# seiya-kumada/3d_gaussian_splatting

Measured on AMD Instinct MI355X. Metric: forward+backward iters/s at 1080p, 1M Gaussians; PSNR vs CPU ref, higher is better.
Workload: dtype f32; 1 GPU; 1m_1080p: 1000000 Gaussians, 1920x1080, SH degree 3, fwd+bwd; gaussians=1000000, width=1920, height=1080, sh_degree=3, parallelism=single GPU

## Files before the change

### 3d_gaussian_splatting_amd/csrc/gsr_api.cpp

```cpp
#include <hip/hip_runtime.h>

#include <algorithm>
#include <climits>
#include <cstdlib>
#include <cstdarg>
#include <cstdio>
#include <cstring>
#include <mutex>
#include <string>
#include <vector>

#include "gsr_kernels.h"

using namespace gsr;

namespace {

thread_local std::string g_err;

struct PinnedWord {
    static constexpr int kWords = 256;
    volatile uint32_t* p = nullptr;
    PinnedWord() {
        void* q = nullptr;
// ... 265 lines not shown
        v.kA = at<uint32_t>(b->binning, bl.kA);
        v.vA = at<uint32_t>(b->binning, bl.vA);
        v.kB = at<uint32_t>(b->binning, bl.kB);
        v.vB = at<uint32_t>(b->binning, bl.vB);
        v.hist = at<uint32_t>(b->binning, bl.hist);
        v.mk = at<uint8_t>(b->binning, bl.mk);
        v.rb_histB = at<uint32_t>(b->binning, bl.rb_hist);
        const int tiles = div_up(cam->width, kTile) * div_up(cam->height, kTile);
        const bool odd = !v.rb && (tile_passes(tiles) & 1) != 0;
        v.sorted_tile = odd ? v.kB : v.kA;
        v.sorted_gid = odd ? v.vB : v.vA;
        v.free_k = odd ? v.kA : v.kB;
        v.free_v = odd ? v.vA : v.vB;
    }
    return v;
}

__global__ void fill_background(float* out_color, float* final_T, float* accum,
                                int npix, float bg0, float bg1, float bg2) {
    const int i = blockIdx.x * 256 + threadIdx.x;
    if (i >= npix) return;
    accum[i] = 0.0f;
    accum[npix + i] = 0.0f;
    accum[2 * (size_t)npix + i] = 0.0f;
    out_color[i] = bg0;
    out_color[npix + i] = bg1;
    out_color[2 * (size_t)npix + i] = bg2;
    final_T[i] = 1.0f;
}

struct FwdJob {
    const gsr_camera* cam;
    const gsr_raster_settings* rs;
    float* out_color;
    gsr_buffers* bufs;
    long long n = 0;
    int ty0 = 0, ty1 = 0, gx = 0, gy = 0;
    int vgy = 0, vh = 0;
    bool rows_counted = false;
    const gsr_aux_out* aux = nullptr;
    bool antialias() const { return (rs->flags & GSR_FLAG_ANTIALIAS) != 0; }
    uint32_t mode_bits() const {
        return (aux ? kBufAux | ((rs->flags & GSR_FLAG_INVDEPTH) ? kBufInvDepth : 0u) : 0u) |
               (antialias() ? kBufAntialias : 0u);
    }
};

template <class Pre>
int fwd_phase1(FwdJob& j, gsr_alloc_fn alloc_geom, gsr_alloc_fn alloc_image, void* ctx, hipStream_t stream, bool debug,
               bool band_pixels_only, Pre&& pre) {
    const gsr_camera* cam = j.cam;
    const gsr_raster_settings* rs = j.rs;
    gsr_buffers* bufs = j.bufs;
    const int W = cam->width, H = cam->height;
    j.gx = div_up(W, kTile);
    j.gy = div_up(H, kTile);
    band(cam, rs, &j.ty0, &j.ty1);
    std::memset(bufs, 0, sizeof *bufs);
    bufs->layout = GSR_LAYOUT_TAG | (use_presort(j.n, j.gx, j.gy) ? kBufPresort : 0u) | j.mode_bits();
    bufs->num_rendered = -1;
    bufs->n_local = (int32_t)j.n;
    bufs->geom = alloc_geom(ctx, GeomLayout(j.n).total);
    bufs->image = alloc_image(ctx, ImgLayout(W, H, j.aux != nullptr).total);
    if (!bufs->geom || !bufs->image) return fail(-2, "allocation failed (geometry/image)");
    const ImgLayout il(W, H);
    const Views v = views(cam, j.n, bufs);
    if ((j.ty0 > 0 || j.ty1 < j.gy) && !band_pixels_only) {
        const int npix = W * H;
        hipLaunchKernelGGL(fill_background, dim3(div_up(npix, 256)), dim3(256), 0, stream, j.out_color, v.final_T,
                           v.accum, npix, rs->bg[0], rs->bg[1], rs->bg[2]);
        GSR_STAGE(GSR_STAGE_MISC, hipGetLastError(), "fill_background");
    }
    GSR_STAGE(GSR_STAGE_MISC, hipMemsetAsync(v.ranges, 0, il.ovf - il.ranges, stream), "clear ranges");
    if (int e = pre(v)) return e;
    if (v.presort) {
        GSR_STAGE(GSR_STAGE_DEPTH_SORT, launch_depth_presort(v.depth_key, v.tiles, v.rect, (int)j.n, v.dk0, v.dv0,
                                                             v.dk1, v.dv1, v.dhist, v.rtiles, v.rrect, v.lookback,
                                                             v.K_dev, stream),
                  "depth presort");
        return 0;
    }
    const bool rb_possible = use_rb_binning(j.n, j.gx, j.gy);
    if (rb_possible && j.rows_counted)
        GSR_STAGE(GSR_STAGE_SCAN, launch_scan_blocks(v.lookback + 16, (int)j.n, v.K_dev, stream), "scan (block sums)");
    else
        GSR_STAGE(GSR_STAGE_SCAN, launch_scan(v.tiles, (int)j.n, v.offsets, v.partials, v.K_dev, stream, !rb_possible),
                  "scan");
    return 0;
}

int fwd_phase2(FwdJob& j, long long cap, gsr_alloc_fn alloc_binning, void* ctx, hipStream_t stream, bool debug) {
    const gsr_camera* cam = j.cam;
    gsr_buffers* bufs = j.bufs;
    if (cap > INT32_MAX) return fail(-3, "num_rendered overflow (%lld)", cap);
    bufs->capacity = (int32_t)cap;
    bufs->binning = alloc_binning(ctx, BinLayout(cap, (long long)ImgLayout::tile_count(cam->width, cam->height),
                                                 j.aux != nullptr).total);
    if (!bufs->binning) return fail(-2, "allocation failed (binning, %lld instances)", cap);
    const int tiles = j.gx * j.gy, ntiles = (j.ty1 - j.ty0) * j.gx;
    const bool scanned = use_rb_binning(j.n, j.gx, j.gy);
    bufs->layout = expected_layout(j.n, j.gx, j.gy, cap) | j.mode_bits();
    const Views v = views(cam, j.n, bufs);
    auto depth_sort = [&](bool unordered, const uint2* src) {
        return launch_tile_depth_sort(v.ranges, j.ty0 * j.gx, ntiles, cap, v.depth_key, v.sorted_gid, v.ovf,
                                      v.counters + kOvfCountSlot, v.ovf2, v.counters + kOvf2CountSlot, v.done,
                                      v.free_k, v.free_v, stream, unordered, src);
    };
    if (v.presort)
        GSR_STAGE(GSR_STAGE_DUPLICATE, launch_duplicate_ranked(v.rtiles, v.rrect, v.rect, (int)j.n, j.gx, j.ty0,
                                                               v.lookback, v.offsets, v.kA, v.vA, cap, stream),
                  "duplicate (rank order)");
    else if (!v.rb) {
        if (scanned && j.rows_counted)
            GSR_STAGE(GSR_STAGE_SCAN, launch_block_offsets(v.tiles, (int)j.n, v.lookback + 16, v.offsets, stream),
                      "offsets");
        GSR_STAGE(GSR_STAGE_DUPLICATE, launch_duplicate(v.tiles, v.rect, (int)j.n, j.gx, j.ty0, v.offsets, v.lookback,
                                                        v.kA, v.vA, cap, v.K_dev, stream, scanned),
                  "duplicate");
    }
    if (cap > 0 && v.rb) {
        const bool rb_keys = v.ck_bytes >= 4 * (size_t)cap;
        uint2* const ppair = rb_keys ? reinterpret_cast<uint2*>(v.kA) : nullptr;
        uint2* const tpair = rb_keys ? reinterpret_cast<uint2*>(v.kB) : nullptr;
        uint32_t* const pxr = rb_keys ? reinterpret_cast<uint32_t*>(v.ck) : v.vB;
        GSR_STAGE(GSR_STAGE_TILE_SORT, launch_rb_binning(v.tiles, v.rect, v.offsets, (int)j.n, j.gx, j.ty0, j.ty1,
                                                         v.rb_histA, v.rb_histB, v.rb_status, v.kB, pxr, v.vA,
                                                         v.ranges, cap, stream, j.rows_counted,
                                                         j.rows_counted ? v.lookback + 16 : nullptr, v.K_dev,
                                                         v.depth_key, ppair, tpair),
                  "row-bucketed binning");
        GSR_STAGE(GSR_STAGE_DEPTH_SORT, depth_sort(true, tpair), "per-tile depth order");
    } else if (cap > 0) {
        int which = -1;
        GSR_STAGE(GSR_STAGE_TILE_SORT, radix_sort(v.kA, v.vA, v.kB, v.vB, v.kA, v.vA, cap, v.K_dev, tile_bits(tiles),
                                                  v.hist, &which, stream),
                  "tile sort");
        if ((which == 0) != (v.sorted_tile == v.kB)) return fail(-12, "tile sort ended in an unexpected buffer");
        GSR_STAGE(GSR_STAGE_FINALIZE, launch_finalize(v.sorted_tile, cap, v.K_dev, v.ranges, stream), "finalize");
        if (!v.presort) GSR_STAGE(GSR_STAGE_DEPTH_SORT, depth_sort(false, nullptr), "per-tile depth order");
    }
    F6Aux f6{};
    if (j.aux)
        f6 = {v.depth_key, j.aux->depth, j.aux->alpha, v.accum_z, v.ckz, (j.rs->flags & GSR_FLAG_INVDEPTH) ? 1 : 0};
    GSR_STAGE(GSR_STAGE_BLEND_FWD, launch_blend_forward(*cam, j.rs->bg, j.ty0, j.ty1, v.ranges, v.sorted_gid, v.rec,
                                                        j.out_color, v.final_T, v.accum, v.term, v.ck, cap, stream,
                                                        j.vgy, j.vh, v.mk, j.aux ? &f6 : nullptr),
              j.aux ? "blend forward (aux)" : "blend forward");
    return 0;
}

int fwd_sized_phase2(FwdJob& j, gsr_alloc_fn alloc_binning, void* ctx, hipStream_t stream, bool debug) {
    long long cap = j.rs->max_rendered;
    if (cap == 0) {
        uint64_t ksum = 0;
        if (j.n > 0) {
            uint32_t cw[2 * kCountSlots];
            const Views v = views(j.cam, j.n, j.bufs);
            GSR_STAGE(GSR_STAGE_MISC, end_read(v.counters, cw, 2 * kCountSlots, stream), "read counts");
            for (int i = 0; i < kCountSlots; ++i) ksum += cw[kCountSlots + i];
        }
        if (ksum > (uint64_t)INT32_MAX) return fail(-3, "num_rendered overflow (%llu)", (unsigned long long)ksum);
        cap = (long long)ksum;
        j.bufs->num_rendered = (int32_t)ksum;
    }
    return fwd_phase2(j, cap, alloc_binning, ctx, stream, debug);
}

// ... 680 lines not shown
```

### 3d_gaussian_splatting_amd/csrc/gsr_binning.hip

```cpp
#include "gsr_kernels.h"
#include "gsr_sort_dev.h"

namespace gsr {
namespace {

constexpr int kB = kSortBlock;
constexpr int kI = kSortItems;
constexpr int kWaves = kB / 64;

__device__ inline uint32_t block_exclusive_scan(uint32_t v, uint32_t* wsum, uint32_t* total) {
    const int tid = threadIdx.x, w = tid >> 6, lane = tid & 63;
    uint32_t x = v;
#pragma unroll
    for (int o = 1; o < 64; o <<= 1) {
        const uint32_t y = __shfl_up(x, o, 64);
        if (lane >= o) x += y;
    }
    if (lane == 63) wsum[w] = x;
    __syncthreads();
    uint32_t pre = 0, tot = 0;
    const int nw = blockDim.x >> 6;
    for (int k = 0; k < nw; ++k) {
        pre += (k < w) ? wsum[k] : 0u;
        tot += wsum[k];
// ... 1 lines not shown
    __syncthreads();
    *total = tot;
    return pre + x - v;
}

__global__ __launch_bounds__(kB) void scan_reduce(const uint32_t* __restrict__ in, int n,
                                                  uint32_t* __restrict__ partials) {
    __shared__ uint32_t wsum[kWaves];
    const int base = blockIdx.x * kSortTile;
    uint32_t s = 0;
#pragma unroll
    for (int r = 0; r < kI; ++r) {
        const int i = base + r * kB + threadIdx.x;
        if (i < n) s += in[i];
    }
    uint32_t tot;
    block_exclusive_scan(s, wsum, &tot);
    if (threadIdx.x == 0) partials[blockIdx.x] = tot;
}

constexpr int kScanQ = 8, kScanQ1 = 32;
__device__ __forceinline__ uint32_t wide_block_scan(uint32_t* __restrict__ a, int n, uint32_t* wsum) {
    uint32_t carry = 0;
    for (int base = 0; base < n; base += 1024 * kScanQ) {
        const int i0 = base + (int)threadIdx.x * kScanQ;
        uint32_t v[kScanQ], sv = 0;
#pragma unroll
        for (int q = 0; q < kScanQ; ++q) {
            v[q] = i0 + q < n ? a[i0 + q] : 0u;
            sv += v[q];
        }
        uint32_t tot;
        uint32_t run = carry + block_exclusive_scan(sv, wsum, &tot);
#pragma unroll
        for (int q = 0; q < kScanQ; ++q) {
            if (i0 + q < n) a[i0 + q] = run;
            run += v[q];
        }
        carry += tot;
    }
    return carry;
}

__device__ __forceinline__ uint32_t wide_block_scan_lds(uint32_t* __restrict__ a, int n, uint32_t* wsum,
                                                        uint32_t* buf) {
    for (int i = (int)threadIdx.x; i < n; i += 1024) buf[i] = a[i];
    __syncthreads();
    const int Q = (n + 1023) / 1024;
    const int i0 = (int)threadIdx.x * Q;
    uint32_t v[kScanQ1], sv = 0;
#pragma unroll
    for (int q = 0; q < kScanQ1; ++q) {
        v[q] = q < Q && i0 + q < n ? buf[i0 + q] : 0u;
        sv += v[q];
    }
    uint32_t tot;
    uint32_t run = block_exclusive_scan(sv, wsum, &tot);
#pragma unroll
    for (int q = 0; q < kScanQ1; ++q) {
        if (q < Q && i0 + q < n) buf[i0 + q] = run;
        run += v[q];
    }
    __syncthreads();
    for (int i = (int)threadIdx.x; i < n; i += 1024) a[i] = buf[i];
    return tot;
}
__host__ __device__ constexpr bool scan_lds_fits(long long n) { return n <= 1024LL * kScanQ1; }

__global__ __launch_bounds__(1024) void scan_partials(uint32_t* __restrict__ partials, int nb,
                                                      uint32_t* __restrict__ total_out) {
    extern __shared__ uint32_t sbuf[];
    __shared__ uint32_t wsum[16];
    const uint32_t carry = scan_lds_fits(nb) ? wide_block_scan_lds(partials, nb, wsum, sbuf)
                                             : wide_block_scan(partials, nb, wsum);
    if (threadIdx.x == 0 && total_out) *total_out = carry;
}

__global__ __launch_bounds__(1024) void rb_colscan(uint32_t* __restrict__ hist, int nb, uint32_t* __restrict__ totals) {
    extern __shared__ uint32_t sbuf[];
    __shared__ uint32_t wsum[16];
    uint32_t* const a = hist + (size_t)blockIdx.x * nb;
    const uint32_t carry = scan_lds_fits(nb) ? wide_block_scan_lds(a, nb, wsum, sbuf) : wide_block_scan(a, nb, wsum);
    if (threadIdx.x == 0) totals[blockIdx.x] = carry;
}
static size_t scan_lds_bytes(long long n) { return scan_lds_fits(n) ? sizeof(uint32_t) * (size_t)n : 0; }

__global__ __launch_bounds__(kB) void scan_downsweep(const uint32_t* __restrict__ in, int n,
                                                     const uint32_t* __restrict__ partials,
                                                     uint32_t* __restrict__ out) {
    __shared__ uint32_t buf[kSortTile + kSortTile / 32];
    __shared__ uint32_t wsum[kWaves];
    const int base = blockIdx.x * kSortTile;
    const int tid = threadIdx.x;
    auto pad = [](int i) { return i + (i >> 5); };
#pragma unroll
    for (int r = 0; r < kI; ++r) {
        const int i = r * kB + tid;
        const int g = base + i;
        buf[pad(i)] = g < n ? in[g] : 0u;
    }
    __syncthreads();
    uint32_t v[kI];
    uint32_t s = 0;
#pragma unroll
    for (int k = 0; k < kI; ++k) {
        v[k] = buf[pad(tid * kI + k)];
        s += v[k];
        v[k] = s;
    }
    uint32_t tot;
    const uint32_t ex = block_exclusive_scan(s, wsum, &tot) + partials[blockIdx.x];
#pragma unroll
    for (int k = 0; k < kI; ++k) buf[pad(tid * kI + k)] = v[k] + ex;
    __syncthreads();
#pragma unroll
    for (int r = 0; r < kI; ++r) {
        const int i = r * kB + tid;
        if (base + i < n) out[base + i] = buf[pad(i)];
    }
}

__device__ __forceinline__ uint32_t udiv_small(uint32_t a, uint32_t b) {
    return (uint32_t)(((float)a + 0.5f) * __builtin_amdgcn_rcpf((float)b));
}

__device__ __forceinline__ void emit_wave(const uint32_t* s_start, const uint32_t* s_g, const uint32_t* s_w,
                                          const uint32_t* s_x0, const uint32_t* s_y0, uint32_t first,
                                          uint32_t wtotal, int grid_x, long long cap, uint32_t* __restrict__ tkey,
                                          uint32_t* __restrict__ tgid) {
    const int lane = threadIdx.x & 63;
    for (uint32_t i = lane; i < wtotal; i += 64) {
        if ((long long)first + i >= cap) break;
        int o = 0;
#pragma unroll
        for (int step = 32; step > 0; step >>= 1)
            if (s_start[o + step] <= i) o += step;
        const uint32_t local = i - s_start[o];
        const uint32_t wd = s_w[o];
        const uint32_t dy = udiv_small(local, wd), dx = local - dy * wd;
        tkey[first + i] = (s_y0[o] + dy) * (uint32_t)grid_x + s_x0[o] + dx;
        tgid[first + i] = s_g[o];
    }
}

constexpr uint32_t kAgg = 1u << 30, kInc = 2u << 30, kCntMask = kAgg - 1u;

__global__ __launch_bounds__(256) void scan_duplicate_kernel(const uint32_t* __restrict__ tiles,
                                                             uint4* __restrict__ rect, int n,
                                                             int grid_x, int ty0,
                                                             uint32_t* __restrict__ offsets,
                                                             uint32_t* __restrict__ tkey,
                                                             uint32_t* __restrict__ tgid, long long cap,
                                                             uint32_t* __restrict__ status,
                                                             uint32_t* __restrict__ ticket,
                                                             uint32_t* __restrict__ total_out) {
    __shared__ uint32_t s_start[kWaves][64], s_g[kWaves][64], s_w[kWaves][64], s_x0[kWaves][64],
        s_y0[kWaves][64];
    __shared__ uint32_t wsum[kWaves];
    __shared__ uint32_t s_excl;
    __shared__ int s_b;
    const int tid = threadIdx.x, w = tid >> 6, lane = tid & 63;
    if (tid == 0) s_b = (int)atomicAdd(ticket, 1u);
    __syncthreads();
    const int b = s_b;
    const int g = b * 256 + tid;
    const bool valid = g < n;
// ... 77 lines not shown
                                                        const uint32_t* __restrict__ tiles,
                                                        uint4* __restrict__ rect, const uint4* __restrict__ rrect,
                                                        int P, int grid_x, int ty0,
                                                        uint32_t* __restrict__ tkey, uint32_t* __restrict__ tgid,
                                                        long long cap, const uint32_t* __restrict__ bexcl) {
    __shared__ uint32_t s_start[kWaves][64], s_g[kWaves][64], s_w[kWaves][64], s_x0[kWaves][64],
        s_y0[kWaves][64];
    __shared__ uint32_t wsum[kWaves];
    const int tid = threadIdx.x, w = tid >> 6, lane = tid & 63;
    const int i = blockIdx.x * 256 + tid;
    const bool valid = i < P;
    uint32_t nt = 0, end = 0, g = (uint32_t)i;
    if (RANKED) {
        if (valid) nt = tiles[i];
        uint32_t tot;
        end = bexcl[blockIdx.x] + block_exclusive_scan(nt, wsum, &tot) + nt;
        if (valid) offsets[i] = end;
    } else if (valid) {
        nt = tiles[i];
        end = offsets[i];
    }
    uint32_t minx = 0, maxx = 0, y0 = 0;
    if (nt) {
        uint4 rr;
        if (RANKED) {
            rr = rrect[i];
            g = rr.z;
            rect[g].z = end - nt;
        } else {
            rect[g].z = end - nt;
            rr = rect[g];
        }
        minx = rr.x & 0xFFFF;
        maxx = rr.y & 0xFFFF;
        const uint32_t miny = rr.x >> 16;
        y0 = miny > (uint32_t)ty0 ? miny : (uint32_t)ty0;
    }
    const uint32_t first = (uint32_t)__builtin_amdgcn_readfirstlane((int)(end - nt));
    const uint64_t vmask = __ballot(valid);
    if (vmask == 0) return;
    const int last_lane = 63 - __builtin_clzll(vmask);
    const uint32_t total = (uint32_t)__builtin_amdgcn_readlane((int)end, last_lane) - first;
    s_start[w][lane] = valid ? end - nt - first : 0xFFFFFFFFu;
    s_g[w][lane] = g;
    s_w[w][lane] = maxx - minx;
    s_x0[w][lane] = minx;
    s_y0[w][lane] = y0;
    wave_lds_sync();
    emit_wave(s_start[w], s_g[w], s_w[w], s_x0[w], s_y0[w], first, total, grid_x, cap, tkey, tgid);
}

__global__ __launch_bounds__(256) void rank_payload_kernel(const uint32_t* __restrict__ sgid,
                                                           const uint32_t* __restrict__ tiles,
                                                           const uint4* __restrict__ rect, int n,
                                                           uint32_t* __restrict__ rtiles,
                                                           uint4* __restrict__ rrect, uint32_t* __restrict__ bsum) {
    __shared__ uint32_t wsum[kWaves];
    const int r = blockIdx.x * 256 + threadIdx.x;
    uint32_t nt = 0;
    if (r < n) {
        const uint32_t g = sgid[r];
        nt = tiles[g];
        uint4 q = make_uint4(0u, 0u, g, 0u);
        if (nt) {
            const uint4 rr = rect[g];
            q.x = rr.x;
            q.y = rr.y;
        }
        rtiles[r] = nt;
        rrect[r] = q;
    }
    uint32_t s = nt;
#pragma unroll
    for (int o = 32; o > 0; o >>= 1) s += __shfl_xor(s, o, 64);
    if ((threadIdx.x & 63) == 0) wsum[threadIdx.x >> 6] = s;
    __syncthreads();
    if (threadIdx.x == 0) bsum[blockIdx.x] = wsum[0] + wsum[1] + wsum[2] + wsum[3];
}

constexpr int kRbChunk = kRbChunkPairs;
static_assert(kRbChunk % 256 == 0 && kRbMaxRows == 256 && kRbMaxCols == 256, "one row / column per thread");
constexpr int kRbStageA = 1024;
constexpr int kRbStage = 4096;

__global__ __launch_bounds__(256) void rb_rows_count(const uint32_t* __restrict__ tiles, const uint4* __restrict__ rect,
                                                     int n, int ty0, int ty1, uint32_t* __restrict__ histA, int nbA) {
    __shared__ uint32_t cnt[kRbMaxRows];
    const int tid = threadIdx.x, R = ty1 - ty0;
    cnt[tid] = 0u;
    __syncthreads();
    const int g = blockIdx.x * 256 + tid;
    if (g < n) {
        const uint32_t nt = tiles[g];
        if (nt) {
            const uint4 rr = rect[g];
            const int miny = (int)(rr.x >> 16), maxy = (int)(rr.y >> 16);
            const int by0 = miny > ty0 ? miny : ty0, by1 = maxy < ty1 ? maxy : ty1;
            for (int r = by0; r < by1; ++r) atomicAdd(&cnt[r - ty0], 1u);
        }
    }
    __syncthreads();
    if (tid < R) histA[(size_t)tid * nbA + blockIdx.x] = cnt[tid];
}

__global__ __launch_bounds__(256) void rb_rows_place(const uint32_t* __restrict__ tiles, uint4* __restrict__ rect,
                                                     uint32_t* __restrict__ offsets, const uint32_t* __restrict__ bsum,
                                                     int n, int ty0, int ty1,
                                                     const uint32_t* __restrict__ histA,
                                                     const uint32_t* __restrict__ totA, int nbA,
                                                     uint32_t* __restrict__ pgid, uint32_t* __restrict__ pxr,
                                                     long long pcap, const uint32_t* __restrict__ depth_key,
                                                     uint2* __restrict__ ppair) {
    __shared__ uint32_t cnt[kRbMaxRows];
    __shared__ uint32_t gb[kRbMaxRows];
    __shared__ uint32_t lb[kRbMaxRows];
    __shared__ uint32_t sg[kRbStageA], sx[kRbStageA], sk[kRbStageA];
    __shared__ uint8_t sr[kRbStageA];
    __shared__ uint32_t wsum[kWaves];
    const int tid = threadIdx.x, R = ty1 - ty0;
    cnt[tid] = 0u;
    const uint32_t ta = tid < R ? totA[tid] : 0u;
    const uint32_t ha = tid < R ? histA[(size_t)tid * nbA + blockIdx.x] : 0u;
    const int g = blockIdx.x * 256 + tid;
    int by0 = 0, by1 = 0;
    uint32_t xr = 0;
    const uint32_t nt = g < n ? tiles[g] : 0u;
    uint32_t incl;
    if (bsum) {
        const uint32_t bb = bsum[blockIdx.x];
        uint32_t tdum;
        incl = bb + block_exclusive_scan(nt, wsum, &tdum) + nt;
        if (g < n) offsets[g] = incl;
    } else {
        incl = g < n ? offsets[g] : 0u;
    }
    if (nt) {
        const uint4 rr = rect[g];
        rect[g].z = incl - nt;
        const int miny = (int)(rr.x >> 16), maxy = (int)(rr.y >> 16);
        by0 = (miny > ty0 ? miny : ty0) - ty0;
        by1 = (maxy < ty1 ? maxy : ty1) - ty0;
        xr = (rr.x & 0xFFFFu) | (rr.y << 16);
    }
    const uint32_t dk = ppair && nt ? depth_key[g] : 0u;
    __syncthreads();
    for (int r = by0; r < by1; ++r) atomicAdd(&cnt[r], 1u);
    __syncthreads();
    uint32_t tot;
    {
        const uint32_t c = cnt[tid];
        uint32_t sdum;
        const uint32_t rowbase = block_exclusive_scan(ta, wsum, &sdum);
        gb[tid] = tid < R ? rowbase + ha : 0u;
        lb[tid] = block_exclusive_scan(c, wsum, &tot);
        cnt[tid] = 0u;
    }
    __syncthreads();
    const bool staged = tot <= (uint32_t)kRbStageA;
    for (int r = by0; r < by1; ++r) {
        const uint32_t k = atomicAdd(&cnt[r], 1u);
        if (staged) {
            sg[lb[r] + k] = (uint32_t)g;
            sx[lb[r] + k] = xr;
            if (ppair) sk[lb[r] + k] = dk;
            sr[lb[r] + k] = (uint8_t)r;
        } else {
// ... 16 lines not shown
            pxr[pos] = sx[i];
        }
    }
}

struct RbRows {
    uint32_t pbase[kRbMaxRows];
    uint32_t cbase[kRbMaxRows];
    uint32_t npair[kRbMaxRows];
    uint32_t wsum[kWaves];
    uint32_t nchunks;
};

__device__ __forceinline__ void rb_rows_table(const uint32_t* __restrict__ totA, int R, long long pcap, RbRows& t) {
    const int tid = threadIdx.x;
    const uint32_t ta = tid < R ? totA[tid] : 0u;
    uint32_t tp;
    const uint32_t pb = block_exclusive_scan(ta, t.wsum, &tp);
    const long long avail = pcap - (long long)pb;
    const uint32_t tc = avail <= 0 ? 0u : (avail < (long long)ta ? (uint32_t)avail : ta);
    uint32_t tcs;
    const uint32_t cb = block_exclusive_scan((tc + kRbChunk - 1) / kRbChunk, t.wsum, &tcs);
    t.pbase[tid] = pb;
    t.cbase[tid] = tid < R ? cb : 0xFFFFFFFFu;
    t.npair[tid] = tc;
    if (tid == 0) t.nchunks = tcs;
    __syncthreads();
}

struct RbChunk {
    int r, k, nch;
    uint32_t p0, p1, cp;
};

__device__ __forceinline__ RbChunk rb_chunk(const RbRows& t, uint32_t b) {
    int r = 0;
#pragma unroll
    for (int step = kRbMaxRows / 2; step > 0; step >>= 1)
        if (t.cbase[r + step] <= b) r += step;
    RbChunk ch;
    ch.r = r;
    ch.cp = t.cbase[r];
    ch.k = (int)(b - ch.cp);
    ch.nch = (int)((t.npair[r] + kRbChunk - 1) / kRbChunk);
    ch.p0 = t.pbase[r] + (uint32_t)ch.k * kRbChunk;
    const uint32_t end = t.pbase[r] + t.npair[r];
    ch.p1 = ch.p0 + kRbChunk < end ? ch.p0 + kRbChunk : end;
    return ch;
}

__global__ __launch_bounds__(256) void rb_chunks_count(const uint32_t* __restrict__ pxr, const uint32_t* __restrict__ totA,
                                                       int R, int gx, long long pcap, uint32_t* __restrict__ histB) {
    __shared__ RbRows t;
    __shared__ uint32_t cnt[kRbMaxCols];
    const int tid = threadIdx.x;
    rb_rows_table(totA, R, pcap, t);
    for (uint32_t b = blockIdx.x; b < t.nchunks; b += gridDim.x) {
        const RbChunk ch = rb_chunk(t, b);
        cnt[tid] = 0u;
        __syncthreads();
#pragma unroll
        for (int q = 0; q < kRbChunk / 256; ++q) {
            const uint32_t p = ch.p0 + q * 256 + tid;
            if (p < ch.p1) {
                const uint32_t xr = pxr[p];
                for (uint32_t c = xr & 0xFFFFu; c < (xr >> 16); ++c) atomicAdd(&cnt[c], 1u);
            }
        }
        __syncthreads();
        if (tid < gx) histB[(size_t)gx * ch.cp + (size_t)tid * ch.nch + ch.k] = cnt[tid];
    }
}

constexpr int kRbScanThreads = 1024, kRbScanQ = 32;
__global__ __launch_bounds__(kRbScanThreads) void rb_tiles_scan(const uint32_t* __restrict__ totA, int R, int gx,
                                                                int ty0, long long pcap, long long cap,
                                                                uint32_t* __restrict__ histB,
                                                                uint32_t* __restrict__ status,
                                                                uint32_t* __restrict__ ticket,
                                                                uint2* __restrict__ ranges,
                                                                uint32_t* __restrict__ K_dev, int G) {
    __shared__ uint32_t wsum[kRbScanThreads / 64];
    __shared__ uint32_t tstart[kRbMaxCols];
    __shared__ uint32_t s_row[2];
    __shared__ int s_p;
    __shared__ uint32_t s_base;
    const int tid = threadIdx.x, lane = tid & 63;
    if (tid == 0) s_p = (int)atomicAdd(ticket, 1u);
    __syncthreads();
    const int p = s_p, r = p / G, gi = p - r * G;
    const int c0 = gi * gx / G, c1 = (gi + 1) * gx / G;
    {
        const uint32_t ta = tid < R ? totA[tid] : 0u;
        uint32_t tp;
        const uint32_t pb = block_exclusive_scan(ta, wsum, &tp);
        const long long avail = pcap - (long long)pb;
        const uint32_t tc = avail <= 0 ? 0u : (avail < (long long)ta ? (uint32_t)avail : ta);
        const uint32_t nc = (tc + kRbChunk - 1) / kRbChunk;
        uint32_t tcs;
        const uint32_t cb = block_exclusive_scan(nc, wsum, &tcs);
        if (tid == r) {
            s_row[0] = nc;
            s_row[1] = cb;
        }
        __syncthreads();
    }
    const uint32_t nch = s_row[0], cp = s_row[1];
    uint32_t* const h = histB + (size_t)gx * cp + (size_t)c0 * nch;
    const uint32_t E = (uint32_t)(c1 - c0) * nch;
    const uint32_t Q = (E + kRbScanThreads - 1) / kRbScanThreads;
    const bool one = Q <= (uint32_t)kRbScanQ;
    const uint32_t i0 = Q * tid;
    uint32_t cnts[kRbScanQ], excl = 0, carry = 0;
    if (one) {
        uint32_t sv = 0;
#pragma unroll
        for (int q = 0; q < kRbScanQ; ++q) {
            cnts[q] = (uint32_t)q < Q && i0 + q < E ? h[i0 + q] : 0u;
            sv += cnts[q];
        }
        excl = block_exclusive_scan(sv, wsum, &carry);
    } else {
        for (uint32_t base = 0; base < E; base += 4 * kRbScanThreads) {
            const uint32_t j0 = base + 4 * tid;
            uint32_t v[4], sv = 0;
#pragma unroll
            for (int q = 0; q < 4; ++q) {
                v[q] = j0 + q < E ? h[j0 + q] : 0u;
                sv += v[q];
            }
            uint32_t tot;
            uint32_t run = carry + block_exclusive_scan(sv, wsum, &tot);
#pragma unroll
            for (int q = 0; q < 4; ++q) {
                if (j0 + q < E) h[j0 + q] = run;
                run += v[q];
            }
            carry += tot;
        }
    }
    if (tid < 64) {
        uint32_t excl = 0;
        if (p == 0) {
            if (lane == 0) __hip_atomic_store(status, kInc | carry, __ATOMIC_RELAXED, __HIP_MEMORY_SCOPE_AGENT);
        } else {
            if (lane == 0) __hip_atomic_store(status + p, kAgg | carry, __ATOMIC_RELAXED, __HIP_MEMORY_SCOPE_AGENT);
            int pos = p - 1;
            uint32_t spins = 0;
            while (true) {
                const int idx = pos - lane;
                uint32_t v = kInc;
                if (idx >= 0) v = __hip_atomic_load(status + idx, __ATOMIC_RELAXED, __HIP_MEMORY_SCOPE_AGENT);
                while (__ballot((v & ~kCntMask) == 0u)) {
                    if (++spins > (1u << 24)) break;
                    __builtin_amdgcn_s_sleep(1);
                    if (idx >= 0 && (v & ~kCntMask) == 0u)
                        v = __hip_atomic_load(status + idx, __ATOMIC_RELAXED, __HIP_MEMORY_SCOPE_AGENT);
                }
                const uint64_t inc = __ballot((v & kInc) != 0u);
                const int k = inc ? __builtin_ctzll(inc) : 64;
                uint32_t c = lane <= k ? (v & kCntMask) : 0u;
#pragma unroll
                for (int o = 32; o > 0; o >>= 1) c += __shfl_xor(c, o, 64);
                excl += c;
                if (inc || spins > (1u << 24)) break;
                pos -= 64;
            }
            if (lane == 0) __hip_atomic_store(status + p, kInc | (excl + carry), __ATOMIC_RELAXED, __HIP_MEMORY_SCOPE_AGENT);
            if (spins > (1u << 24) && lane == 0 && K_dev) *K_dev = 0xFFFFFFFFu;
        }
        if (lane == 0) s_base = excl;
    }
    __syncthreads();
    const uint32_t pbase = s_base;
    if (one) {
        uint32_t run = pbase + excl;
        uint32_t c = i0 / (nch ? nch : 1u), k = i0 - c * nch;
#pragma unroll
        for (int q = 0; q < kRbScanQ; ++q) {
            if ((uint32_t)q < Q && i0 + q < E) {
                h[i0 + q] = run;
                if (k == 0) tstart[c0 + c] = run;
                run += cnts[q];
                if (++k == nch) k = 0, ++c;
            }
        }
    } else {
        for (uint32_t i = tid; i < E; i += kRbScanThreads) h[i] += pbase;
        __syncthreads();
        if (tid >= c0 && tid < c1 && nch) tstart[tid] = h[(size_t)(tid - c0) * nch];
    }
    __syncthreads();
    if (tid >= c0 && tid < c1) {
        const uint32_t a = nch ? tstart[tid] : pbase, e = tid + 1 < c1 && nch ? tstart[tid + 1] : pbase + carry;
        const long long a2 = a < cap ? a : cap, e2 = e < cap ? e : cap;
        ranges[(size_t)(ty0 + r) * gx + tid] = e2 > a2 ? make_uint2((uint32_t)a2, (uint32_t)e2) : make_uint2(0u, 0u);
    }
}

constexpr int kRbPlaceWpe = 1;
__global__ __launch_bounds__(256) __attribute__((amdgpu_waves_per_eu(kRbPlaceWpe))) void rb_chunks_place(const uint32_t* __restrict__ pgid, const uint32_t* __restrict__ pxr,
                                                       const uint32_t* __restrict__ totA, int R, int gx,
                                                       long long pcap, long long cap,
                                                       const uint32_t* __restrict__ histB,
                                                       uint32_t* __restrict__ tgid,
                                                       const uint2* __restrict__ ppair,
                                                       uint2* __restrict__ tpair) {
    __shared__ RbRows t;
    __shared__ uint32_t cnt[kRbMaxCols];
    __shared__ uint32_t lb[kRbMaxCols];
    __shared__ uint32_t gb[kRbMaxCols];
    __shared__ uint32_t pg[kRbChunk], pk[kRbChunk];
    __shared__ uint32_t spc[kRbStage];
    __shared__ uint32_t wsum[kWaves];
    static_assert(kRbChunk <= 65536, "u16 pair index");
    const int tid = threadIdx.x;
    const bool keys = tpair != nullptr;
    rb_rows_table(totA, R, pcap, t);
    constexpr int kQ = kRbChunk / 256;
    uint32_t nxr[kQ], ngg[kQ], nkk[kQ];
    auto load_pairs = [&](uint32_t b) {
        const RbChunk c = rb_chunk(t, b);
#pragma unroll
        for (int q = 0; q < kQ; ++q) {
            const uint32_t p = c.p0 + q * 256 + tid;
            nxr[q] = p < c.p1 ? pxr[p] : 0u;
            if (keys) {
                const uint2 pp = p < c.p1 ? ppair[p] : make_uint2(0u, 0u);
                ngg[q] = pp.x;
                nkk[q] = pp.y;
            } else {
                ngg[q] = p < c.p1 ? pgid[p] : 0u;
                nkk[q] = 0u;
            }
        }
    };
    if (blockIdx.x < t.nchunks) load_pairs(blockIdx.x);
    for (uint32_t b = blockIdx.x; b < t.nchunks; b += gridDim.x) {
        const RbChunk ch = rb_chunk(t, b);
        cnt[tid] = 0u;
        const uint32_t hb = tid < gx ? histB[(size_t)gx * ch.cp + (size_t)tid * ch.nch + ch.k] : 0u;
        uint32_t xr[kQ], gg[kQ], kk[kQ];
#pragma unroll
        for (int q = 0; q < kQ; ++q) {
            xr[q] = nxr[q];
            gg[q] = ngg[q];
            kk[q] = nkk[q];
        }
        if (b + gridDim.x < t.nchunks) load_pairs(b + gridDim.x);
        __syncthreads();
#pragma unroll
        for (int q = 0; q < kQ; ++q)
            for (uint32_t c = xr[q] & 0xFFFFu; c < (xr[q] >> 16); ++c) atomicAdd(&cnt[c], 1u);
        __syncthreads();
        uint32_t tot;
        {
            const uint32_t c = cnt[tid];
            lb[tid] = block_exclusive_scan(c, wsum, &tot);
            gb[tid] = hb;
            cnt[tid] = 0u;
        }
        __syncthreads();
        const bool staged = tot <= (uint32_t)kRbStage;
        if (staged) {
#pragma unroll
            for (int q = 0; q < kQ; ++q) {
                pg[q * 256 + tid] = gg[q];
                if (keys) pk[q * 256 + tid] = kk[q];
            }
        }
#pragma unroll
        for (int q = 0; q < kQ; ++q) {
            for (uint32_t c = xr[q] & 0xFFFFu; c < (xr[q] >> 16); ++c) {
                const uint32_t k = atomicAdd(&cnt[c], 1u);
                if (staged) {
                    spc[lb[c] + k] = (uint32_t)(q * 256 + tid) | (c << 16);
                } else {
                    const long long pos = (long long)gb[c] + k;
                    if (pos < cap) {
                        if (keys) tpair[pos] = make_uint2(gg[q], kk[q]);
                        else tgid[pos] = gg[q];
                    }
                }
            }
        }
        if (staged) {
            __syncthreads();
            for (int i = tid; i < (int)tot; i += 256) {
                const uint32_t pc = spc[i];
                const int c = (int)(pc >> 16);
                const long long pos = (long long)gb[c] + ((uint32_t)i - lb[c]);
                if (pos < cap) {
                    const int pi = (int)(pc & 0xFFFFu);
                    if (keys) tpair[pos] = make_uint2(pg[pi], pk[pi]);
                    else tgid[pos] = pg[pi];
                }
            }
        }
        __syncthreads();
    }
}

constexpr int kFinQ = 4;
__global__ __launch_bounds__(256) void finalize_kernel(const uint32_t* __restrict__ stile, long long cap,
                                                       const uint32_t* __restrict__ n_dev,
                                                       uint2* __restrict__ ranges) {
    const long long K = live_count(cap, n_dev);
    const long long i0 = ((long long)blockIdx.x * 256 + threadIdx.x) * kFinQ;
    if (i0 >= K) return;
    uint32_t t[kFinQ];
    if (i0 + kFinQ <= K) {
        const uint4 q = *reinterpret_cast<const uint4*>(stile + i0);
        t[0] = q.x, t[1] = q.y, t[2] = q.z, t[3] = q.w;
    } else {
#pragma unroll
        for (int j = 0; j < kFinQ; ++j) t[j] = i0 + j < K ? stile[i0 + j] : 0xFFFFFFFFu;
    }
    uint32_t prev = i0 > 0 ? stile[i0 - 1] : 0xFFFFFFFFu;
#pragma unroll
    for (int j = 0; j < kFinQ; ++j) {
        const long long i = i0 + j;
        if (i >= K) break;
        const uint32_t next = j + 1 < kFinQ ? t[j + 1] : (i + 1 < K ? stile[i + 1] : 0xFFFFFFFFu);
        if (i == 0 || prev != t[j]) ranges[t[j]].x = (uint32_t)i;
        if (i == K - 1 || next != t[j]) ranges[t[j]].y = (uint32_t)(i + 1);
        prev = t[j];
    }
}

}

int launch_scan(const uint32_t* tiles, int n, uint32_t* offsets, uint32_t* scan_partials_buf, uint32_t* total_out,
                hipStream_t s, bool fused_ok) {
    if (n <= 0) return (int)hipMemsetAsync(total_out, 0, sizeof(uint32_t), s);
    if (fused_ok && n <= kFusedScanMax) return 0;
    const int nb = sort_blocks(n);
    hipLaunchKernelGGL(scan_reduce, dim3(nb), dim3(kB), 0, s, tiles, n, scan_partials_buf);
    hipLaunchKernelGGL(scan_partials, dim3(1), dim3(1024), scan_lds_bytes(nb), s, scan_partials_buf, nb, total_out);
    hipLaunchKernelGGL(scan_downsweep, dim3(nb), dim3(kB), 0, s, tiles, n, scan_partials_buf, offsets);
    return (int)hipGetLastError();
}

__global__ __launch_bounds__(256) void block_offsets_kernel(const uint32_t* __restrict__ tiles, int n,
                                                            const uint32_t* __restrict__ bsum,
                                                            uint32_t* __restrict__ offsets) {
    __shared__ uint32_t wsum[kWaves];
    const int g = blockIdx.x * 256 + threadIdx.x;
    const uint32_t nt = g < n ? tiles[g] : 0u;
    uint32_t tdum;
    const uint32_t incl = bsum[blockIdx.x] + block_exclusive_scan(nt, wsum, &tdum) + nt;
    if (g < n) offsets[g] = incl;
}

int launch_scan_blocks(uint32_t* bsum, int n, uint32_t* total_out, hipStream_t s) {
    if (n <= 0) return (int)hipMemsetAsync(total_out, 0, sizeof(uint32_t), s);
    hipLaunchKernelGGL(scan_partials, dim3(1), dim3(1024), scan_lds_bytes(div_up(n, 256)), s, bsum, div_up(n, 256),
                       total_out);
    return (int)hipGetLastError();
}

int launch_block_offsets(const uint32_t* tiles, int n, const uint32_t* bsum, uint32_t* offsets, hipStream_t s) {
    if (n <= 0) return 0;
    hipLaunchKernelGGL(block_offsets_kernel, dim3(div_up(n, 256)), dim3(256), 0, s, tiles, n, bsum, offsets);
    return (int)hipGetLastError();
}

int launch_rb_binning(const uint32_t* tiles, uint4* rect, uint32_t* offsets, int n, int gx, int ty0, int ty1,
                      uint32_t* histA, uint32_t* histB, uint32_t* rb_status, uint32_t* pgid, uint32_t* pxr,
                      uint32_t* tgid, uint2* ranges, long long cap, hipStream_t s,
                      bool rows_counted, const uint32_t* bsum, uint32_t* K_dev, const uint32_t* depth_key,
                      uint2* ppair, uint2* tpair) {
    const int R = ty1 - ty0;
    if (!depth_key || !ppair || !tpair) ppair = tpair = nullptr;
    if (n <= 0 || R <= 0 || cap <= 0) return 0;
    if (R > kRbMaxRows || gx > kRbMaxCols || cap >= kRbMaxCap) return (int)hipErrorInvalidValue;
    const int nbA = div_up(n, 256);
    uint32_t* const totA = histA + (size_t)256 * nbA;
    if (!rows_counted)
        hipLaunchKernelGGL(rb_rows_count, dim3(nbA), dim3(256), 0, s, tiles, rect, n, ty0, ty1, histA, nbA);
    hipLaunchKernelGGL(rb_colscan, dim3(R), dim3(1024), scan_lds_bytes(nbA), s, histA, nbA, totA);
    hipLaunchKernelGGL(rb_rows_place, dim3(nbA), dim3(256), 0, s, tiles, rect, offsets, bsum, n, ty0, ty1, histA, totA,
                       nbA, pgid, pxr, cap, depth_key, ppair);
    const int nch_max = div_up(cap, kRbChunk) + R;
    const int gcount = nch_max < 2048 ? nch_max : 2048, gplace = nch_max < 1280 ? nch_max : 1280;
    hipLaunchKernelGGL(rb_chunks_count, dim3(gcount), dim3(256), 0, s, pxr, totA, R, gx, cap, histB);
    int G = kRbScanSplit < 256 / R ? kRbScanSplit : 256 / R;
    G = G < 1 ? 1 : G > gx ? gx : G;
    hipLaunchKernelGGL(rb_tiles_scan, dim3(R * G), dim3(kRbScanThreads), 0, s, totA, R, gx, ty0, cap, cap, histB,
                       rb_status + 16, rb_status, ranges, K_dev, G);
    hipLaunchKernelGGL(rb_chunks_place, dim3(gplace), dim3(256), 0, s, pgid, pxr, totA, R, gx, cap, cap, histB,
                       tgid, ppair, tpair);
    return (int)hipGetLastError();
}

int launch_duplicate(const uint32_t* tiles, uint4* rect, int n, int grid_x, int ty0, uint32_t* offsets,
                     uint32_t* lookback, uint32_t* tkey, uint32_t* tgid, long long cap, uint32_t* total_out,
                     hipStream_t s, bool scanned) {
    if (n <= 0) return 0;
    if (n <= kFusedScanMax && !scanned) {
        const int nb = div_up(n, 256);
        if (hipError_t e = hipMemsetAsync(lookback, 0, sizeof(uint32_t) * (16 + (size_t)nb), s)) return (int)e;
        hipLaunchKernelGGL(scan_duplicate_kernel, dim3(nb), dim3(256), 0, s, tiles, rect, n, grid_x, ty0, offsets,
                           tkey, tgid, cap, lookback + 16, lookback, total_out);
        return (int)hipGetLastError();
    }
    hipLaunchKernelGGL(duplicate_kernel<false>, dim3(div_up(n, 256)), dim3(256), 0, s, offsets, tiles, rect,
                       nullptr, n, grid_x, ty0, tkey, tgid, cap, nullptr);
    return (int)hipGetLastError();
}

int launch_depth_presort(const uint32_t* depth_key, const uint32_t* tiles, const uint4* rect, int n, uint32_t* dk0,
                         uint32_t* dv0, uint32_t* dk1, uint32_t* dv1, uint32_t* hist, uint32_t* rtiles, uint4* rrect,
                         uint32_t* bsum, uint32_t* total_out, hipStream_t s) {
    if (n <= 0) return (int)hipMemsetAsync(total_out, 0, sizeof(uint32_t), s);
    int which = -1;
    if (int e = radix_sort(depth_key, nullptr, dk0, dv0, dk1, dv1, n, nullptr, 32, hist, &which, s)) return e;
    const uint32_t* sgid = which == 0 ? dv0 : dv1;
    const int nb = div_up(n, 256);
    hipLaunchKernelGGL(rank_payload_kernel, dim3(nb), dim3(256), 0, s, sgid, tiles, rect, n, rtiles, rrect, bsum);
    hipLaunchKernelGGL(scan_partials, dim3(1), dim3(1024), scan_lds_bytes(nb), s, bsum, nb, total_out);
    return (int)hipGetLastError();
}

int launch_duplicate_ranked(const uint32_t* rtiles, const uint4* rrect, uint4* rect, int n, int grid_x, int ty0,
                            const uint32_t* bexcl, uint32_t* offsets, uint32_t* tkey, uint32_t* tgid, long long cap,
                            hipStream_t s) {
    if (n <= 0) return 0;
    hipLaunchKernelGGL(duplicate_kernel<true>, dim3(div_up(n, 256)), dim3(256), 0, s, offsets, rtiles, rect, rrect, n,
                       grid_x, ty0, tkey, tgid, cap, bexcl);
    return (int)hipGetLastError();
}

__global__ __launch_bounds__(256) void tile_keys_from_ranges(const uint2* __restrict__ ranges, long long cap,
                                                             uint32_t* __restrict__ tkey) {
    const uint2 rg = ranges[blockIdx.x];
    const uint32_t e = rg.y < cap ? rg.y : (uint32_t)cap;
    for (uint32_t i = rg.x + threadIdx.x; i < e; i += 256) tkey[i] = blockIdx.x;
}

int launch_tile_keys_from_ranges(const uint2* ranges, int tiles, long long cap, uint32_t* tkey, hipStream_t s) {
    if (tiles <= 0 || cap <= 0) return 0;
    hipLaunchKernelGGL(tile_keys_from_ranges, dim3(tiles), dim3(256), 0, s, ranges, cap, tkey);
    return (int)hipGetLastError();
}

int launch_finalize(const uint32_t* sorted_tile, long long cap, const uint32_t* K_dev, uint2* ranges, hipStream_t s) {
    if (cap <= 0) return 0;
    hipLaunchKernelGGL(finalize_kernel, dim3(div_up(div_up(cap, kFinQ), 256)), dim3(256), 0, s, sorted_tile, cap, K_dev,
                       ranges);
    return (int)hipGetLastError();
}

}
```

### 3d_gaussian_splatting_amd/csrc/gsr_kernels.h

```cpp
#pragma once
#include <hip/hip_runtime.h>

#include "gsr_internal.h"

namespace gsr {

struct GaussIn {
    int P, D, M_rest;
    float smod;
    const float *means3D, *sh_dc, *sh_rest, *colors, *opac, *scales, *rots, *cov3D;
};

struct PreOut {
    int32_t* radii;
    uint32_t* depth_key;
    uint32_t* tiles;
    float4* rec;
    uint4* rect;
    uint32_t* flags;
    uint32_t* counters;
    uint32_t* rb_hist = nullptr;
    uint32_t* bsum = nullptr;
};

int launch_preprocess(const gsr_camera& cam, const GaussIn& in, int ty0, int ty1, const PreOut& out,
                      hipStream_t s, bool aa = false);
template <int NV>
struct CamArg {
    gsr_camera c[NV];
};
int launch_preprocess_views(const gsr_camera* cams, int V, const GaussIn& in, const PreOut& out, hipStream_t s,
                            bool aa = false);

int radix_sort(const uint32_t* keys_in, const uint32_t* vals_in, uint32_t* k0, uint32_t* v0,
               uint32_t* k1, uint32_t* v1, long long cap, const uint32_t* n_dev, int nbits, uint32_t* hist,
               int* which, hipStream_t s);

int launch_scan(const uint32_t* tiles, int n, uint32_t* offsets, uint32_t* scan_partials_buf, uint32_t* total_out,
                hipStream_t s, bool fused_ok = true);
int launch_duplicate(const uint32_t* tiles, uint4* rect, int n, int grid_x, int ty0, uint32_t* offsets,
                     uint32_t* lookback, uint32_t* tkey, uint32_t* tgid, long long cap, uint32_t* total_out,
                     hipStream_t s, bool scanned = false);

int launch_scan_blocks(uint32_t* bsum, int n, uint32_t* total_out, hipStream_t s);
int launch_block_offsets(const uint32_t* tiles, int n, const uint32_t* bsum, uint32_t* offsets, hipStream_t s);
int launch_rb_binning(const uint32_t* tiles, uint4* rect, uint32_t* offsets, int n, int gx, int ty0, int ty1,
                      uint32_t* histA, uint32_t* histB, uint32_t* rb_status, uint32_t* pgid, uint32_t* pxr,
                      uint32_t* tgid, uint2* ranges, long long cap, hipStream_t s,
                      bool rows_counted = false,
                      const uint32_t* bsum = nullptr,
                      uint32_t* K_dev = nullptr,
                      const uint32_t* depth_key = nullptr,
                      uint2* ppair = nullptr,
                      uint2* tpair = nullptr);

int launch_depth_presort(const uint32_t* depth_key, const uint32_t* tiles, const uint4* rect, int n, uint32_t* dk0,
                         uint32_t* dv0, uint32_t* dk1, uint32_t* dv1, uint32_t* hist, uint32_t* rtiles, uint4* rrect,
                         uint32_t* bsum, uint32_t* total_out, hipStream_t s);
int launch_duplicate_ranked(const uint32_t* rtiles, const uint4* rrect, uint4* rect, int n, int grid_x, int ty0,
                            const uint32_t* bexcl, uint32_t* offsets, uint32_t* tkey, uint32_t* tgid, long long cap,
                            hipStream_t s);

int launch_finalize(const uint32_t* sorted_tile, long long cap, const uint32_t* K_dev, uint2* ranges, hipStream_t s);
int launch_tile_keys_from_ranges(const uint2* ranges, int tiles, long long cap, uint32_t* tkey, hipStream_t s);

int launch_tile_depth_sort(const uint2* ranges, int tile0, int ntiles, long long K, const uint32_t* depth_key,
                           uint32_t* gid, uint32_t* ovf, uint32_t* ovf_count, uint32_t* ovf2, uint32_t* ovf2_count,
                           uint32_t* done, uint32_t* scratch_hi, uint32_t* scratch_lo, hipStream_t s,
                           bool unordered = false, const uint2* src = nullptr);

struct F6Aux {
    const uint32_t* depth_key;
    float *out_depth, *out_alpha;
    float *accum_z, *ckz;
    int inv;
};
struct B1Aux {
    const uint32_t* depth_key;
    const float *accum_z, *dL_ddepth, *dL_dalpha, *ckz;
    float* pz;
    int inv;
};

int launch_blend_forward(const gsr_camera& cam, const float bg[3], int ty0, int ty1,
                         const uint2* ranges, const uint32_t* sorted_gid, const float4* rec,
                         float* out_color, float* final_T, float* accum, uint32_t* term, float4* ck, long long cap,
                         hipStream_t s, int vgy = 0, int vh = 0, uint8_t* mk = nullptr, const F6Aux* aux = nullptr);

int launch_clear_flags(float* partial, long long cap, bool aux, hipStream_t s);
int launch_blend_backward(const gsr_camera& cam, const float bg[3], int ty0, int ty1,
                          const uint2* ranges, const uint32_t* sorted_gid, const uint4* rect,
                          const float4* rec, const float* final_T,
                          const float* accum, const float* dL_dpix, float* partial, long long cap,
                          const uint32_t* term, const float4* ck, hipStream_t s, int vgy = 0, int vh = 0,
                          const uint8_t* mk = nullptr, const B1Aux* aux = nullptr);

constexpr float kLn2 = 0.6931471805599453f;

int launch_gather_grad2d(const uint32_t* offsets, const float* partial, const float4* rec, int W, int H,
                         long long cap, int P, const uint4* rrect, float* grad2d, hipStream_t s,
                         bool aux = false);

struct GradOut {
    float *means2D, *conic, *opac, *colors, *means3D, *sh_dc, *sh_rest, *scales, *rots, *cov3D;
};

int launch_preprocess_backward(const gsr_camera& cam, const GaussIn& in, int g0, int g1,
                               const uint32_t* depth_key, const uint32_t* flags, const float* grad2d,
                               const GradOut& out, hipStream_t s, int aux = 0, bool aa = false);
int launch_preprocess_backward_views(const gsr_camera* cams, int V, const GaussIn& in, const uint32_t* depth_key,
                                     const uint32_t* flags, const float* grad2d, const GradOut& out,
                                     const GradOut& scratch, hipStream_t s, bool aa = false);
int launch_views_sum(const GaussIn& in, int V, const GradOut& out, const GradOut& scratch, hipStream_t s);

int launch_pack_splats(const uint32_t* tiles, const uint4* rect, const uint32_t* depth_key, const float4* rec, int P,
                       const BandRows& br, uint32_t* partials, char* send, int pair_cap, uint32_t* slot_of,
                       uint32_t* row_hist, int grid_y, bool spans, hipStream_t s, uint32_t* rowpart = nullptr);
int launch_unpack_splats(const char* recv, int nsrc, int pair_cap, int ty0, int ty1, float4* rec, uint32_t* depth_key,
                         uint32_t* tiles, uint4* rect, hipStream_t s, uint32_t* rb_hist = nullptr,
                         uint32_t* bsum = nullptr);

int launch_band_publish(const float* color, int W, int H, int py0, int py1, int tall, float* mine,
                        long long status_off, const char* send, size_t block_bytes, int nbands, const uint32_t* K_dev,
                        hipStream_t s);
int launch_gather_finish(const float* gathered, long long row_floats, long long status_off, int world,
                         const BandRows& br, int W, int H, int tall, float* image, uint32_t pair_cap,
                         uint32_t capacity, int32_t* guard, float* zero, int nzero, hipStream_t s);
// ... 25 lines not shown
```

Measured before the change: 926.4 iters/s.

## Fuse row column-scan into block-sum scan and reuse histB in place pass

The per-row column scan of histA is merged into the block-sum scan launch as extra blocks, so it runs in phase 1 instead of as a separate launch during binning. The tiles scan also writes a sentinel end entry into histB, which lets the chunk placement kernel read per-column counts from consecutive histB entries. That removes its LDS atomic recount pass and two block barriers. This saves a kernel launch and redundant atomics, but relies on histB prefix entries being contiguous and the sentinel being correct.

```diff
diff --git a/3d_gaussian_splatting_amd/csrc/gsr_api.cpp b/3d_gaussian_splatting_amd/csrc/gsr_api.cpp
--- a/3d_gaussian_splatting_amd/csrc/gsr_api.cpp
+++ b/3d_gaussian_splatting_amd/csrc/gsr_api.cpp
@@ -371,7 +371,9 @@
     }
     const bool rb_possible = use_rb_binning(j.n, j.gx, j.gy);
     if (rb_possible && j.rows_counted)
-        GSR_STAGE(GSR_STAGE_SCAN, launch_scan_blocks(v.lookback + 16, (int)j.n, v.K_dev, stream), "scan (block sums)");
+        GSR_STAGE(GSR_STAGE_SCAN, launch_scan_blocks_rows(v.lookback + 16, (int)j.n, v.K_dev, v.rb_histA,
+                                                          j.ty1 > j.ty0 ? j.ty1 - j.ty0 : 0, stream),
+                  "scan (block sums, row counts)");
     else
         GSR_STAGE(GSR_STAGE_SCAN, launch_scan(v.tiles, (int)j.n, v.offsets, v.partials, v.K_dev, stream, !rb_possible),
                   "scan");
diff --git a/3d_gaussian_splatting_amd/csrc/gsr_binning.hip b/3d_gaussian_splatting_amd/csrc/gsr_binning.hip
--- a/3d_gaussian_splatting_amd/csrc/gsr_binning.hip
+++ b/3d_gaussian_splatting_amd/csrc/gsr_binning.hip
@@ -107,6 +107,16 @@
     uint32_t* const a = hist + (size_t)blockIdx.x * nb;
     const uint32_t carry = scan_lds_fits(nb) ? wide_block_scan_lds(a, nb, wsum, sbuf) : wide_block_scan(a, nb, wsum);
     if (threadIdx.x == 0) totals[blockIdx.x] = carry;
+}
+__global__ __launch_bounds__(1024) void rb_colscan_blocks(uint32_t* __restrict__ hist, int nb, uint32_t* __restrict__ totals,
+                                                          int R, uint32_t* __restrict__ bsum,
+                                                          uint32_t* __restrict__ total_out) {
+    extern __shared__ uint32_t sbuf[];
+    __shared__ uint32_t wsum[16];
+    const bool sums = (int)blockIdx.x == R;
+    uint32_t* const a = sums ? bsum : hist + (size_t)blockIdx.x * nb;
+    const uint32_t carry = scan_lds_fits(nb) ? wide_block_scan_lds(a, nb, wsum, sbuf) : wide_block_scan(a, nb, wsum);
+    if (threadIdx.x == 0) *(sums ? total_out : totals + blockIdx.x) = carry;
 }
 static size_t scan_lds_bytes(long long n) { return scan_lds_fits(n) ? sizeof(uint32_t) * (size_t)n : 0; }
 
@@ -350,6 +360,7 @@
 static_assert(kRbChunk % 256 == 0 && kRbMaxRows == 256 && kRbMaxCols == 256, "one row / column per thread");
 constexpr int kRbStageA = 1024;
 constexpr int kRbStage = 4096;
+constexpr int kRbCountGrid = 2048, kRbPlaceGrid = 1280;
 
 __global__ __launch_bounds__(256) void rb_rows_count(const uint32_t* __restrict__ tiles, const uint4* __restrict__ rect,
                                                      int n, int ty0, int ty1, uint32_t* __restrict__ histA, int nbA) {
@@ -532,7 +543,7 @@
                                                                 uint32_t* __restrict__ K_dev, int G) {
     __shared__ uint32_t wsum[kRbScanThreads / 64];
     __shared__ uint32_t tstart[kRbMaxCols];
-    __shared__ uint32_t s_row[2];
+    __shared__ uint32_t s_row[3];
     __shared__ int s_p;
     __shared__ uint32_t s_base;
     const int tid = threadIdx.x, lane = tid & 63;
@@ -552,6 +563,7 @@
         if (tid == r) {
             s_row[0] = nc;
             s_row[1] = cb;
+            s_row[2] = tcs;
         }
         __syncthreads();
     }
@@ -623,6 +635,7 @@
     }
     __syncthreads();
     const uint32_t pbase = s_base;
+    if (p == (int)gridDim.x - 1 && tid == 0) histB[(size_t)gx * s_row[2]] = pbase + carry;
     if (one) {
         uint32_t run = pbase + excl;
         uint32_t c = i0 / (nch ? nch : 1u), k = i0 - c * nch;
@@ -668,9 +681,14 @@
     const bool keys = tpair != nullptr;
     rb_rows_table(totA, R, pcap, t);
     constexpr int kQ = kRbChunk / 256;
-    uint32_t nxr[kQ], ngg[kQ], nkk[kQ];
+    uint32_t nxr[kQ], ngg[kQ], nkk[kQ], nhb = 0, nhn = 0;
     auto load_pairs = [&](uint32_t b) {
         const RbChunk c = rb_chunk(t, b);
+        if (tid < gx) {
+            const uint32_t* const h = histB + (size_t)gx * c.cp + (size_t)tid * c.nch + c.k;
+            nhb = h[0];
+            nhn = h[1];
+        }
 #pragma unroll
         for (int q = 0; q < kQ; ++q) {
             const uint32_t p = c.p0 + q * 256 + tid;
@@ -688,8 +706,7 @@
     if (blockIdx.x < t.nchunks) load_pairs(blockIdx.x);
     for (uint32_t b = blockIdx.x; b < t.nchunks; b += gridDim.x) {
         const RbChunk ch = rb_chunk(t, b);
-        cnt[tid] = 0u;
-        const uint32_t hb = tid < gx ? histB[(size_t)gx * ch.cp + (size_t)tid * ch.nch + ch.k] : 0u;
+        const uint32_t hb = nhb, ccol = nhn - nhb;
         uint32_t xr[kQ], gg[kQ], kk[kQ];
 #pragma unroll
         for (int q = 0; q < kQ; ++q) {
@@ -698,18 +715,10 @@
             kk[q] = nkk[q];
         }
         if (b + gridDim.x < t.nchunks) load_pairs(b + gridDim.x);
-        __syncthreads();
-#pragma unroll
-        for (int q = 0; q < kQ; ++q)
-            for (uint32_t c = xr[q] & 0xFFFFu; c < (xr[q] >> 16); ++c) atomicAdd(&cnt[c], 1u);
-        __syncthreads();
         uint32_t tot;
-        {
-            const uint32_t c = cnt[tid];
-            lb[tid] = block_exclusive_scan(c, wsum, &tot);
-            gb[tid] = hb;
-            cnt[tid] = 0u;
-        }
+        lb[tid] = block_exclusive_scan(ccol, wsum, &tot);
+        gb[tid] = hb;
+        cnt[tid] = 0u;
         __syncthreads();
         const bool staged = tot <= (uint32_t)kRbStage;
         if (staged) {
@@ -802,10 +811,12 @@
     if (g < n) offsets[g] = incl;
 }
 
-int launch_scan_blocks(uint32_t* bsum, int n, uint32_t* total_out, hipStream_t s) {
+int launch_scan_blocks_rows(uint32_t* bsum, int n, uint32_t* total_out, uint32_t* histA, int R, hipStream_t s) {
     if (n <= 0) return (int)hipMemsetAsync(total_out, 0, sizeof(uint32_t), s);
-    hipLaunchKernelGGL(scan_partials, dim3(1), dim3(1024), scan_lds_bytes(div_up(n, 256)), s, bsum, div_up(n, 256),
-                       total_out);
+    if (R < 0 || R > kRbMaxRows) return (int)hipErrorInvalidValue;
+    const int nbA = div_up(n, 256);
+    hipLaunchKernelGGL(rb_colscan_blocks, dim3(R + 1), dim3(1024), scan_lds_bytes(nbA), s, histA, nbA,
+                       histA + (size_t)256 * nbA, R, bsum, total_out);
     return (int)hipGetLastError();
 }
 
@@ -826,13 +837,15 @@
     if (R > kRbMaxRows || gx > kRbMaxCols || cap >= kRbMaxCap) return (int)hipErrorInvalidValue;
     const int nbA = div_up(n, 256);
     uint32_t* const totA = histA + (size_t)256 * nbA;
-    if (!rows_counted)
+    if (!rows_counted) {
         hipLaunchKernelGGL(rb_rows_count, dim3(nbA), dim3(256), 0, s, tiles, rect, n, ty0, ty1, histA, nbA);
-    hipLaunchKernelGGL(rb_colscan, dim3(R), dim3(1024), scan_lds_bytes(nbA), s, histA, nbA, totA);
+        hipLaunchKernelGGL(rb_colscan, dim3(R), dim3(1024), scan_lds_bytes(nbA), s, histA, nbA, totA);
+    }
     hipLaunchKernelGGL(rb_rows_place, dim3(nbA), dim3(256), 0, s, tiles, rect, offsets, bsum, n, ty0, ty1, histA, totA,
                        nbA, pgid, pxr, cap, depth_key, ppair);
     const int nch_max = div_up(cap, kRbChunk) + R;
-    const int gcount = nch_max < 2048 ? nch_max : 2048, gplace = nch_max < 1280 ? nch_max : 1280;
+    const int gcount = nch_max < kRbCountGrid ? nch_max : kRbCountGrid;
+    const int gplace = nch_max < kRbPlaceGrid ? nch_max : kRbPlaceGrid;
     hipLaunchKernelGGL(rb_chunks_count, dim3(gcount), dim3(256), 0, s, pxr, totA, R, gx, cap, histB);
     int G = kRbScanSplit < 256 / R ? kRbScanSplit : 256 / R;
     G = G < 1 ? 1 : G > gx ? gx : G;
diff --git a/3d_gaussian_splatting_amd/csrc/gsr_kernels.h b/3d_gaussian_splatting_amd/csrc/gsr_kernels.h
--- a/3d_gaussian_splatting_amd/csrc/gsr_kernels.h
+++ b/3d_gaussian_splatting_amd/csrc/gsr_kernels.h
@@ -42,7 +42,7 @@
                      uint32_t* lookback, uint32_t* tkey, uint32_t* tgid, long long cap, uint32_t* total_out,
                      hipStream_t s, bool scanned = false);
 
-int launch_scan_blocks(uint32_t* bsum, int n, uint32_t* total_out, hipStream_t s);
+int launch_scan_blocks_rows(uint32_t* bsum, int n, uint32_t* total_out, uint32_t* histA, int R, hipStream_t s);
 int launch_block_offsets(const uint32_t* tiles, int n, const uint32_t* bsum, uint32_t* offsets, hipStream_t s);
 int launch_rb_binning(const uint32_t* tiles, uint4* rect, uint32_t* offsets, int n, int gx, int ty0, int ty1,
                       uint32_t* histA, uint32_t* histB, uint32_t* rb_status, uint32_t* pgid, uint32_t* pxr,
```

New measurement: 934.6 iters/s (median of 6 runs). No clear change (+0.9%).
